# cqf7419/LiDAR-GS

Hardware: AMD Instinct MI355X
Metric: LiDAR range-view frames/sec (fwd+bwd) (higher is better)
Workload: dtype f32

## Files before the change

### lidar-gs_amd/csrc/api.hip

```cpp
#include "lidargs_common.h"
#include "../../include/lidargs_rasterizer.h"

#include <math.h>
#include <stdio.h>
#include <stdlib.h>
#include <string.h>
#include <limits>
#include <algorithm>
#include <mutex>

namespace {
using lg::SegPlan;

thread_local char g_err[512] = "";
thread_local long long g_counters[10] = {0, 0, 0, 0, 0, 0, 0, 0, -1, -1};
thread_local int g_counters_on = 0;
struct CounterPage {
    unsigned long long* dev = nullptr; unsigned long long* host = nullptr; hipEvent_t done = nullptr; int device = -1; bool pending = false;
    bool ready() {
        int d = -1;
        if (hipGetDevice(&d) != hipSuccess) return false;
        if (dev && d == device) return true;
        if (dev) { (void)hipFree(dev); dev = nullptr; }
        if (done) { (void)hipEventDestroy(done); done = nullptr; }
// ... 435 lines not shown
    lg::BinnedFrame bf;
    const int rendered = lg::bin_frame(spec, geom, img.ranges, (size_t)P, width, height, col_lo, col_hi, pp.compact != 0, binning_alloc, binning_user,
                                       debug, stream, &bf);
    if (rendered < 0) return rendered;
    const lg::FrameLayout& L = bf.L;
    const lg::BinView& bin = bf.bin;
    const size_t R = bf.R;

    lg::RenderFwdArgs ra;
    ra.fill.cnt = nullptr;
    ra.grid = L.grid; ra.ranges = img.ranges; ra.point_list = bin.val_a; ra.rec = geom.rec; ra.rowspan = geom.rowspan;
    ra.coltab = img.coltab; ra.rowtab = img.rowtab; ra.bg = background; ra.T_in = T_in;
    ra.final_T = img.final_T; ra.T_pass = T_out;
    ra.out_color = out_color; ra.out_depth = out_depth; ra.out_occ = out_occ;
    ra.seg = bin.seg; ra.S = L.S; ra.seg_len = L.plan.seg_len;
    ra.run_pass1 = (L.S > 1 || transmittance_pass || is_shell) ? 1 : 0;
    ra.flags = ra.run_pass1 ? bin.flags : nullptr; ra.R = L.Rp;
    ra.touched = geom.touched;
    ra.transmittance_only = transmittance_pass;
    ra.seg_lo = 0; ra.seg_hi = L.S; ra.front = 0; ra.alive = nullptr;
    int head = 0;
    if (!L.fused && !ra.run_pass1 && R) lg::launch_touch_all(geom.touched, radii, (size_t)P, stream);
    if (L.fused) {
        ra.flags = bin.flags; ra.alive = bin.alive;
        lg::launch_render_fused(ra, stream);
        LG_STAGE_CHECK("render fused");
        lg::prof_mark("render_fused", stream);
    } else {
    if (ra.run_pass1) {
        run_pass1_rounds(ra, L.plan, bin.alive, stream, transmittance_pass ? nullptr : &head);
        LG_STAGE_CHECK("render pass 1");
        lg::prof_mark("render_pass1", stream);
    }
    ra.seg_lo = head; ra.seg_hi = L.S;
    if (!transmittance_pass) {
        lg::launch_render_pass2(ra, stream);
        LG_STAGE_CHECK("render pass 2");
        lg::prof_mark("render_pass2", stream);
    }
    if (L.work_list) ra.fill = lg::work_list(bin);
    lg::launch_render_combine(ra, stream);
    LG_STAGE_CHECK("render combine");
    lg::prof_mark("render_combine", stream);
    }

    lg::RenderBwdArgs v = lg::RenderBwdArgs();
    v.walk.cnt = nullptr; v.grid = L.grid; v.ranges = img.ranges; v.seg = bin.seg; v.S = L.S; v.seg_len = L.plan.seg_len; v.R = L.Rp;
    v.alive = L.gated ? bin.alive : nullptr;
    v.flags = L.flags ? bin.flags : nullptr;
    lg::note_forward((size_t)P, R, L, geom.totals, ra.flags, geom.touched, (R != 0 && !transmittance_pass) ? &v : nullptr, stream);
    return rendered;
}

struct BackMode {
    bool is_shell = false;
    const float* behind = nullptr;
    const float* T_final_global = nullptr;
    int col_lo = -1, col_hi = -1;
};

int backward_impl(int P, int R, const float* background, int width, int height, const float* means3D,
                  const float* colors_precomp, const float* scales, float scale_modifier, const float* rotations,
                  const float* cov3D_precomp, const float* viewmatrix, const float* beams, const int* radii, char* geom_buffer,
                  char* binning_buffer, char* image_buffer, const BackMode& mode, const float* dL_dpix, const float* dL_dout_depth, const float* dL_dout_occ, float* dL_dmean2D,
                  float* dL_dconic, float* dL_dopacity, float* dL_dcolor, float* dL_ddepths, float* dL_dmean3D,
                  float* dL_dsphere_means3D, float* dL_dbasis_u1, float* dL_dbasis_u2, float* dL_dcov3D, float* dL_dscale,
                  float* dL_drot, int debug, hipStream_t stream) {
    (void)colors_precomp; (void)beams;
    const int col_lo = mode.col_lo, col_hi = mode.col_hi;
    if (P < 0 || R < 0 || width <= 0 || height <= 0) return fail(LIDARGS_ERR_INVALID_ARGUMENT, "backward: bad sizes%s");
    if (P == 0) return 0;
    if (!geom_buffer || !binning_buffer || !image_buffer) return fail(LIDARGS_ERR_STATE, "backward: missing forward buffers%s");
    if (!means3D || !viewmatrix || !radii || !dL_dpix || !dL_dout_depth || !dL_dout_occ || !dL_dmean2D ||
        !dL_dopacity || !dL_dcolor || !dL_dmean3D || !dL_dscale || !dL_drot || (cov3D_precomp && !dL_dcov3D))
        return fail(LIDARGS_ERR_INVALID_ARGUMENT, "backward: NULL required pointer%s");

    lg::GeomView geom; lg::geom_carve(geom_buffer, (size_t)P, lg::GAUSS_BUFFERS, &geom);
    if (col_lo >= 0 && (col_lo % LG_TILE_W || col_hi <= col_lo || col_hi > width)) return fail(LIDARGS_ERR_INVALID_ARGUMENT, "backward: bad column wedge%s");
    const lg::FrameLayout L = lg::frame_layout(R, width, height, col_lo, col_hi, mode.is_shell ? lg::FRAME_SHELL : lg::FRAME_GAUSS);
    lg::BinView bin; L.bin_carve(binning_buffer, &bin);
    lg::ImgView img; lg::img_carve(image_buffer, width, height, lg::make_grid(width, height, 4).num_tiles(), &img);
    lg::prof_begin(stream, 1);

    lg::ZeroRows zr;
    zr.add(dL_dmean2D, 4); zr.add(dL_dconic, 4); zr.add(dL_dopacity, 1); zr.add(dL_dcolor, 2); zr.add(dL_ddepths, 1); zr.add(dL_dmean3D, 3);
    zr.add(dL_dsphere_means3D, 3); zr.add(dL_dbasis_u1, 3); zr.add(dL_dbasis_u2, 3); zr.add(dL_dcov3D, 6); zr.add(dL_dscale, 3); zr.add(dL_drot, 4);
    lg::launch_zero_touched(geom.touched, reinterpret_cast<float4*>(geom.gacc), 4, (size_t)P, geom.tlist, geom.tcount, zr, stream);
    lg::prof_mark("bwd_zero", stream);

    lg::RenderBwdArgs rb;
    rb.walk.cnt = nullptr;
    rb.grid = L.grid; rb.ranges = img.ranges; rb.point_list = bin.val_a; rb.rec = geom.rec; rb.rowspan = geom.rowspan;
    rb.coltab = img.coltab; rb.rowtab = img.rowtab; rb.bg = background; rb.final_T = img.final_T;
    rb.seg = bin.seg; rb.S = L.S; rb.seg_len = L.plan.seg_len;
    rb.alive = L.gated ? bin.alive : nullptr;
    rb.flags = L.flags ? bin.flags : nullptr; rb.R = L.Rp;
    rb.T_final_global = mode.T_final_global; rb.behind = mode.behind;
    rb.dL_dpix = dL_dpix; rb.dL_ddepth = dL_dout_depth; rb.dL_docc = dL_dout_occ; rb.gacc = geom.gacc;
    if (L.work_list) rb.walk = lg::work_list(bin);
    lg::launch_render_backward(rb, stream);
    LG_STAGE_CHECK("render backward");
    lg::prof_mark("render_bwd", stream);

    lg::GaussBwdArgs gb;
    gb.P = P; gb.scale_modifier = scale_modifier;
    gb.view = viewmatrix;
    gb.means3D = means3D; gb.scales = scales; gb.rotations = rotations; gb.cov3D_precomp = cov3D_precomp; gb.radii = radii;
    gb.gacc = geom.gacc; gb.tlist = geom.tlist; gb.tcount = geom.tcount;
    gb.dL_dmean2D = dL_dmean2D; gb.dL_dconic = dL_dconic; gb.dL_dopacity = dL_dopacity; gb.dL_dcolor = dL_dcolor;
    gb.dL_ddepths = dL_ddepths; gb.dL_dbasis_u1 = dL_dbasis_u1; gb.dL_dbasis_u2 = dL_dbasis_u2;
    gb.dL_dsphere = dL_dsphere_means3D; gb.dL_dmean3D = dL_dmean3D; gb.dL_dcov3D = dL_dcov3D; gb.dL_dscale = dL_dscale;
    gb.dL_drot = dL_drot;
    lg::launch_gaussian_backward(gb, stream);
    LG_STAGE_CHECK("gaussian backward");
    lg::prof_mark("gaussian_bwd", stream);
    return 0;
}

}

extern "C" {

int lidargs_abi_version(void) { return LIDARGS_ABI_VERSION; }
const char* lidargs_last_error(void) { return g_err; }

int lidargs_forward(lidargs_alloc_fn geometry_alloc, void* geometry_user, lidargs_alloc_fn binning_alloc, void* binning_user,
                    lidargs_alloc_fn image_alloc, void* image_user, int P, int D, int M, const float* background, int width,
                    int height, const float* means3D, const float* shs, const float* colors_precomp, const float* opacities,
                    const float* scales, float scale_modifier, const float* rotations, const float* cov3D_precomp,
                    const float* viewmatrix, const float* projmatrix, const float* cam_pos, const float* beam_inclinations,
                    int prefiltered, int lidar_far, int lidar_near, float* out_color, float* out_depth, float* out_occ,
                    int* radii, int* radii_xy, int debug, void* stream) {
    (void)D; (void)M; (void)shs; (void)projmatrix; (void)cam_pos; (void)prefiltered;
    const float inf = std::numeric_limits<float>::infinity();
    return forward_impl(geometry_alloc, geometry_user, binning_alloc, binning_user, image_alloc, image_user, P, background, width,
                        height, means3D, colors_precomp, opacities, scales, scale_modifier, rotations, cov3D_precomp, viewmatrix,
                        beam_inclinations, (float)lidar_near, (float)lidar_far, -inf, inf, nullptr, 0, out_color, out_depth,
                        out_occ, nullptr, radii, radii_xy, debug, (hipStream_t)stream, FrameMode());
}

int lidargs_forward_enqueue(lidargs_alloc_fn geometry_alloc, void* geometry_user, lidargs_alloc_fn binning_alloc, void* binning_user,
                            lidargs_alloc_fn image_alloc, void* image_user, int P, int D, int M, const float* background, int width,
                            int height, const float* means3D, const float* shs, const float* colors_precomp, const float* opacities,
                            const float* scales, float scale_modifier, const float* rotations, const float* cov3D_precomp,
                            const float* viewmatrix, const float* projmatrix, const float* cam_pos, const float* beam_inclinations,
                            int prefiltered, int lidar_far, int lidar_near, float* out_color, float* out_depth, float* out_occ,
                            int* radii, int* radii_xy, int debug, int instance_capacity, int tile_rows, unsigned* status_host, void* stream) {
    (void)D; (void)M; (void)shs; (void)projmatrix; (void)cam_pos; (void)prefiltered;
    if (instance_capacity <= 0) return fail(LIDARGS_ERR_INVALID_ARGUMENT, "forward_enqueue: instance_capacity must be positive%s");
    const float inf = std::numeric_limits<float>::infinity();
    FrameMode mode;
    mode.instance_capacity = instance_capacity; mode.fixed_tile_rows = tile_rows; mode.status_host = status_host;
    return forward_impl(geometry_alloc, geometry_user, binning_alloc, binning_user, image_alloc, image_user, P, background, width,
                        height, means3D, colors_precomp, opacities, scales, scale_modifier, rotations, cov3D_precomp, viewmatrix,
                        beam_inclinations, (float)lidar_near, (float)lidar_far, -inf, inf, nullptr, 0, out_color, out_depth,
                        out_occ, nullptr, radii, radii_xy, debug, (hipStream_t)stream, mode);
}

int lidargs_backward(int P, int D, int M, int R, const float* background, int width, int height, const float* means3D,
                     const float* shs, const float* colors_precomp, const float* scales, float scale_modifier,
                     const float* rotations, const float* cov3D_precomp, const float* viewmatrix, const float* projmatrix,
                     const float* campos, const float* beam_inclinations, float tan_fovx, float tan_fovy, const int* radii,
                     char* geom_buffer, char* binning_buffer, char* image_buffer, const float* dL_dpix,
                     const float* dL_dout_depth, const float* dL_dout_occ, float* dL_dmean2D, float* dL_dconic,
                     float* dL_dopacity, float* dL_dcolor, float* dL_ddepths, float* dL_dmean3D, float* dL_dsphere_means3D,
                     float* dL_dbasis_u1, float* dL_dbasis_u2, float* dL_dcov3D, float* dL_dsh, float* dL_dscale, float* dL_drot,
                     int debug, void* stream) {
    (void)D; (void)M; (void)shs; (void)projmatrix; (void)campos; (void)tan_fovx; (void)tan_fovy; (void)dL_dsh;
    return backward_impl(P, R, background, width, height, means3D, colors_precomp, scales, scale_modifier, rotations, cov3D_precomp,
                         viewmatrix, beam_inclinations, radii, geom_buffer, binning_buffer, image_buffer, BackMode(), dL_dpix,
                         dL_dout_depth, dL_dout_occ, dL_dmean2D, dL_dconic, dL_dopacity, dL_dcolor, dL_ddepths, dL_dmean3D,
                         dL_dsphere_means3D, dL_dbasis_u1, dL_dbasis_u2, dL_dcov3D, dL_dscale, dL_drot, debug, (hipStream_t)stream);
}

int lidargs_visible_filter(lidargs_alloc_fn geometry_alloc, void* geometry_user, lidargs_alloc_fn binning_alloc, void* binning_user,
                           lidargs_alloc_fn image_alloc, void* image_user, int P, int M, int width, int height,
                           const float* means3D, const float* scales, float scale_modifier, const float* rotations,
                           const float* cov3D_precomp, const float* viewmatrix, const float* projmatrix, const float* cam_pos,
                           const float* beam_inclinations, float tan_fovx, float tan_fovy, int prefiltered, int lidar_far,
                           int lidar_near, int* radii, int* radii_xy, int debug, void* stream_) {
    (void)geometry_alloc; (void)geometry_user; (void)binning_alloc; (void)binning_user; (void)image_alloc; (void)image_user;
    (void)M; (void)projmatrix; (void)cam_pos; (void)tan_fovx; (void)tan_fovy; (void)prefiltered;
    hipStream_t stream = (hipStream_t)stream_;
    if (P < 0 || width <= 0 || height < 2) return fail(LIDARGS_ERR_INVALID_ARGUMENT, "visible_filter: bad sizes%s");
    if (P == 0) return 0;
    if (!means3D || !viewmatrix || !beam_inclinations || !radii)
        return fail(LIDARGS_ERR_INVALID_ARGUMENT, "visible_filter: NULL required pointer%s");
    if (!cov3D_precomp && (!scales || !rotations)) return fail(LIDARGS_ERR_INVALID_ARGUMENT, "visible_filter: need scales+rotations or cov3D_precomp%s");
    const lg::TileGrid grid = lg::make_grid(width, height, lg::tile_rows());
    lg::PreprocessParams pp;
    pp.P = P; pp.W = width; pp.H = height; pp.TH = grid.TH; pp.tiles_x = grid.tiles_x; pp.tiles_y = grid.tiles_y;
    pp.scale_modifier = scale_modifier;
    pp.near_f = (float)lidar_near; pp.far_f = (float)lidar_far;
    pp.shell_lo = -std::numeric_limits<float>::infinity(); pp.shell_hi = std::numeric_limits<float>::infinity();
    pp.tile_x_lo = 0; pp.tile_x_hi = grid.tiles_x; pp.compact = 0; pp.prune = 1;
// ... 251 lines not shown
```

### lidar-gs_amd/csrc/lidargs_common.h

```cpp
#pragma once
#include <hip/hip_runtime.h>
#include <stdint.h>
#include <stddef.h>

#define LG_TILE_W 16
#define LG_WAVE_ROWS 4
#define LG_CHANNELS 2

#define LG_SEG_TPASS 0
#define LG_SEG_C0 1
#define LG_SEG_C1 2
#define LG_SEG_D 3
#define LG_SEG_TEND 4
#define LG_SEG_TBREAK 5
#define LG_SEG_LAST 6
#define LG_SEG_PLANES 7

#define LG_REGION 256

namespace lg {

struct Carver {
    char* p;
    explicit Carver(char* base) : p(base) {}
// ... 306 lines not shown
    patch = patches - 1 - patch;
    return patch >= 0 && seg < S;
#elif defined(LG_PATCH_ORDER) && LG_PATCH_ORDER == 2
    seg = (int)(b / (unsigned)patches); patch = (int)(b % (unsigned)patches);
    return seg < S;
#endif
    return patch < patches && seg < S;
}
inline unsigned segment_grid(int patches, int S) { return (unsigned)patches * ((unsigned)S | 1u); }
#endif


__device__ __forceinline__ int segment_count(uint2 range, int S, int seg_len) {
    const uint32_t L = range.y - range.x;
    const uint32_t want = (L + (uint32_t)seg_len - 1u) / (uint32_t)seg_len;
    return (int)min((uint32_t)S, max(1u, want));
}
__device__ __forceinline__ uint2 segment_range(uint2 range, int St, int seg) {
    const uint32_t L = range.y - range.x;
    const uint32_t len = (L + (uint32_t)St - 1u) / (uint32_t)St;
    const uint32_t a = min(range.y, range.x + (uint32_t)seg * len);
    const uint32_t b = min(range.y, a + len);
    return make_uint2(a, b);
}

#endif

struct RenderFwdArgs {
    TileGrid grid;
    const uint2* ranges; const uint32_t* point_list; const float4* rec; const uint32_t* rowspan;
    const float2* coltab; const float2* rowtab;
    const float* bg;
    const float* T_in;
    float* final_T; float* T_pass;
    float* out_color; float* out_depth; float* out_occ;
    float* seg; int S;
    int seg_len;
    uint8_t* flags; size_t R;
    uint8_t* touched = nullptr;
    int seg_lo, seg_hi;
    int front;
    uint8_t* alive;
    int run_pass1;
    int transmittance_only;
    WorkList fill;
    int walk2;
    float* T_end_out = nullptr;
};
void launch_render_pass1(const RenderFwdArgs& a, hipStream_t s);
void launch_render_pass2(const RenderFwdArgs& a, hipStream_t s);
void launch_render_head(const RenderFwdArgs& a, int head, hipStream_t s);
void launch_render_alive(const RenderFwdArgs& a, hipStream_t s);
void launch_render_combine(const RenderFwdArgs& a, hipStream_t s);
void launch_render_fused(const RenderFwdArgs& a, hipStream_t s);

struct RenderBwdArgs {
    TileGrid grid;
    const uint2* ranges; const uint32_t* point_list; const float4* rec; const uint32_t* rowspan;
    const float2* coltab; const float2* rowtab;
    const float* bg;
    const float* final_T;
    const float* seg; int S; int seg_len;
    const uint8_t* flags; size_t R;
    const uint8_t* alive;
    const float* T_final_global;
    const float* behind;
    const float* dL_dpix; const float* dL_ddepth; const float* dL_docc;
    float* gacc;
    WorkList walk;
};
void launch_render_backward(const RenderBwdArgs& a, hipStream_t s);
void launch_count_backward_entries(const RenderBwdArgs& a, unsigned long long* out, hipStream_t s);
void note_forward(size_t P, size_t R, const FrameLayout& L, const uint32_t* totals, const uint8_t* flags, const uint8_t* touched,
                  const RenderBwdArgs* view, hipStream_t s);

struct GaussBwdArgs {
    int P; float scale_modifier; const float* view;
    const float* means3D; const float* scales; const float* rotations; const float* cov3D_precomp; const int* radii;
    const float* gacc;
    const uint8_t* tlist; const uint16_t* tcount;
    float* dL_dmean2D; float* dL_dconic; float* dL_dopacity; float* dL_dcolor; float* dL_ddepths;
    float* dL_dbasis_u1; float* dL_dbasis_u2;
    float* dL_dsphere; float* dL_dmean3D; float* dL_dcov3D; float* dL_dscale; float* dL_drot;
};
void launch_gaussian_backward(const GaussBwdArgs& a, hipStream_t s);

#ifdef __HIPCC__
typedef float row4 __attribute__((ext_vector_type(4), aligned(4)));
typedef float row3 __attribute__((ext_vector_type(3), aligned(4)));
typedef float row2 __attribute__((ext_vector_type(2), aligned(4)));
#if defined(LG_GB_VARIANT) && LG_GB_VARIANT == 5
__device__ __forceinline__ void put4(float* p, size_t i, float x, float y, float z, float w) { if (x != x || w * 0.f != 0.f) *reinterpret_cast<row4*>(p + 4 * i) = row4{x, y, z, w}; }
__device__ __forceinline__ void put3(float* p, size_t i, float x, float y, float z) { if (x != x || z * 0.f != 0.f) *reinterpret_cast<row3*>(p + 3 * i) = row3{x, y, z}; }
__device__ __forceinline__ void put2(float* p, size_t i, float x, float y) { if (x != x || y * 0.f != 0.f) *reinterpret_cast<row2*>(p + 2 * i) = row2{x, y}; }
#else
__device__ __forceinline__ void put4(float* p, size_t i, float x, float y, float z, float w) { *reinterpret_cast<row4*>(p + 4 * i) = row4{x, y, z, w}; }
__device__ __forceinline__ void put3(float* p, size_t i, float x, float y, float z) { *reinterpret_cast<row3*>(p + 3 * i) = row3{x, y, z}; }
__device__ __forceinline__ void put2(float* p, size_t i, float x, float y) { *reinterpret_cast<row2*>(p + 2 * i) = row2{x, y}; }
#endif
#if defined(LG_GB_VARIANT) && LG_GB_VARIANT == 6
__device__ __forceinline__ float3 get3(const float* p, size_t i) { const float f = 1.f + (float)(i & 1023) * 1e-3f; return make_float3(f, 0.5f * f, 0.25f + f); }
__device__ __forceinline__ float4 get4(const float* p, size_t i) { const float f = 1.f + (float)(i & 1023) * 1e-3f; return make_float4(0.5f, 0.5f * f, 0.5f, 0.5f / f); }
#else
__device__ __forceinline__ float3 get3(const float* p, size_t i) { const row3 v = *reinterpret_cast<const row3*>(p + 3 * i); return make_float3(v.x, v.y, v.z); }
__device__ __forceinline__ float4 get4(const float* p, size_t i) { const row4 v = *reinterpret_cast<const row4*>(p + 4 * i); return make_float4(v.x, v.y, v.z, v.w); }
#endif

typedef float v4f __attribute__((ext_vector_type(4)));
typedef float v3f __attribute__((ext_vector_type(3)));
#define LG_LDS_VOLATILE(T) const volatile __attribute__((address_space(3))) T*
__device__ __forceinline__ float4 lds_ahead(const float4* p) {
    const v4f v = *(LG_LDS_VOLATILE(v4f))p;
    return make_float4(v.x, v.y, v.z, v.w);
}
__device__ __forceinline__ float lds_ahead(const float* p) { return *(LG_LDS_VOLATILE(float))p; }
__device__ __forceinline__ uint32_t lds_ahead(const uint32_t* p) { return *(LG_LDS_VOLATILE(uint32_t))p; }

__device__ __forceinline__ float fold_halves32(float a, float b) {
    const auto r = __builtin_amdgcn_permlane32_swap(__float_as_uint(a), __float_as_uint(b), false, false);
    return __uint_as_float(r[0]) + __uint_as_float(r[1]);
}
__device__ __forceinline__ float fold_halves16(float a, float b) {
    const auto r = __builtin_amdgcn_permlane16_swap(__float_as_uint(a), __float_as_uint(b), false, false);
    return __uint_as_float(r[0]) + __uint_as_float(r[1]);
}

__device__ __forceinline__ float plane_product(float T, const float* first, size_t stride, int n) {
    int k = 0;
    for (; k + 8 <= n; k += 8) {
        float x[8];
#pragma unroll
        for (int i = 0; i < 8; i++) x[i] = first[(size_t)(k + i) * stride];
#pragma unroll
        for (int i = 0; i < 8; i++) T *= x[i];
    }
    float x[8];
#pragma unroll
    for (int i = 0; i < 8; i++) x[i] = (k + i < n) ? first[(size_t)(k + i) * stride] : 1.f;
#pragma unroll
    for (int i = 0; i < 8; i++) if (k + i < n) T *= x[i];
    return T;
}
template <int NP>
__device__ __forceinline__ void plane_sums(float (&acc)[NP], const float* first, size_t stride, const int (&plane)[NP], int n) {
    int k = 0;
    for (; k + 4 <= n; k += 4) {
        float x[4][NP];
#pragma unroll
        for (int i = 0; i < 4; i++)
#pragma unroll
            for (int p = 0; p < NP; p++) x[i][p] = first[(size_t)(k + i) * stride + (size_t)plane[p] * 64];
#pragma unroll
        for (int i = 0; i < 4; i++)
#pragma unroll
            for (int p = 0; p < NP; p++) acc[p] += x[i][p];
    }
    for (; k < n; k++)
#pragma unroll
        for (int p = 0; p < NP; p++) acc[p] += first[(size_t)k * stride + (size_t)plane[p] * 64];
}

__device__ __forceinline__ float4 rows_opacity(uint32_t span, float opacity, int y0) {
    const int lo = (int)(span & 0xFFFFu), hi = (int)(span >> 16);
    float4 o;
    o.x = (y0 >= lo && y0 < hi) ? opacity : 0.f;
    o.y = (y0 + 1 >= lo && y0 + 1 < hi) ? opacity : 0.f;
// ... 8 lines not shown
```

### lidar-gs_amd/csrc/preprocess.hip

```cpp
#include "lidargs_common.h"
#include "selection.h"
#include <algorithm>

namespace lg {

__device__ __forceinline__ float3 f3(float x, float y, float z) { return make_float3(x, y, z); }
__device__ __forceinline__ float dot3(float3 a, float3 b) { return a.x * b.x + a.y * b.y + a.z * b.z; }
__device__ __forceinline__ float3 scale3(float3 a, float s) { return f3(a.x * s, a.y * s, a.z * s); }
__device__ __forceinline__ float3 add3(float3 a, float3 b) { return f3(a.x + b.x, a.y + b.y, a.z + b.z); }

__device__ __forceinline__ float3 view_to_world(const float* vm, float3 v) {
    return f3(vm[0] * v.x + vm[1] * v.y + vm[2] * v.z,
              vm[4] * v.x + vm[5] * v.y + vm[6] * v.z,
              vm[8] * v.x + vm[9] * v.y + vm[10] * v.z);
}
__device__ __forceinline__ float3 world_to_view_dir(const float* vm, float3 v) {
    return f3(vm[0] * v.x + vm[4] * v.y + vm[8] * v.z,
              vm[1] * v.x + vm[5] * v.y + vm[9] * v.z,
              vm[2] * v.x + vm[6] * v.y + vm[10] * v.z);
}

struct Sym3 { float xx, xy, xz, yy, yz, zz; };
__device__ __forceinline__ float3 symmul(const Sym3& S, float3 v) {
    return f3(S.xx * v.x + S.xy * v.y + S.xz * v.z,
// ... 243 lines not shown
    {
        __shared__ uint32_t s_part[4][8];
        uint32_t s4 = t4, s8 = t8, s16 = t16, s32 = t32, sv = reftiles ? 1u : 0u, sr = reftiles;
        uint32_t kinv = ~key, kmx = (key == 0xFFFFFFFFu) ? 0u : key;
#pragma unroll
        for (int o = 32; o > 0; o >>= 1) {
            s4 += __shfl_xor(s4, o); s8 += __shfl_xor(s8, o); s16 += __shfl_xor(s16, o); s32 += __shfl_xor(s32, o);
            sv += __shfl_xor(sv, o); sr += __shfl_xor(sr, o);
            kinv = max(kinv, (uint32_t)__shfl_xor((int)kinv, o)); kmx = max(kmx, (uint32_t)__shfl_xor((int)kmx, o));
        }
        if ((threadIdx.x & 63) == 0) {
            uint32_t* q = s_part[threadIdx.x >> 6];
            q[0] = s4; q[1] = s8; q[2] = s16; q[3] = s32; q[4] = sv; q[5] = sr; q[6] = kinv; q[7] = kmx;
        }
        __syncthreads();
        if (threadIdx.x == 6 || threadIdx.x == 7) {
            const int c = threadIdx.x;
            const uint32_t m = max(max(s_part[0][c], s_part[1][c]), max(s_part[2][c], s_part[3][c]));
            if (m) atomicMax(a.key_span + 2 * (size_t)(blockIdx.x % LG_INST_SLOTS) + (c - 6), m);
        }
        if (threadIdx.x < 6) {
            const uint32_t sum = s_part[0][threadIdx.x] + s_part[1][threadIdx.x] + s_part[2][threadIdx.x] + s_part[3][threadIdx.x];
            const size_t slot = (size_t)(blockIdx.x % LG_INST_SLOTS);
            if (sum) {
                if (threadIdx.x < 4) atomicAdd(a.inst_slots + slot * 4 + threadIdx.x, (unsigned long long)sum);
                else atomicAdd(a.diag_slots + slot * 2 + (threadIdx.x - 4), (unsigned long long)sum);
            }
        }
    }
    if (!in_range) return;
    a.touched[idx] = 0;
    a.dkey[idx] = key;
    if (pp.compact) reinterpret_cast<uint32_t*>(a.spans)[idx] = span_pack(rspan, tiles ? xsp : 0u);
    else a.spans[idx] = make_uint4(rspan, tiles ? xsp : 0u, 0u, 0u);
    if (live && tiles) {
        a.rowspan[idx] = rspan;
        float4* r = a.rec + 4 * (size_t)idx;
        r[0] = r0; r[1] = r1; r[2] = r2; r[3] = r3;
    }
}

void launch_preprocess(const PreprocessParams& pp, const float* means3D, const float* scales, const float* rotations,
                       const float* opacities, const float* colors, const float* cov3D_precomp, const float* beams,
                       int* radii, int* radii_xy, GeomView g, const ImgView* tables, bool filter_only, hipStream_t s) {
    PreKernelArgs a;
    a.pp = pp;
    a.means3D = means3D; a.scales = scales; a.rotations = rotations; a.opacities = opacities; a.colors = colors;
    a.cov3D_precomp = cov3D_precomp; a.beams = beams; a.radii = radii; a.radii_xy = radii_xy;
    a.coltab = tables ? tables->coltab : nullptr; a.rowtab = tables ? tables->rowtab : nullptr;
    a.rec = g.rec; a.rowspan = g.rowspan; a.spans = g.spans; a.dkey = g.key_a; a.ids = g.id_a;
    a.touched = g.touched;
    a.inst_slots = reinterpret_cast<unsigned long long*>(g.totals + LG_TOTALS_SLOT_WORD);
    a.diag_slots = reinterpret_cast<unsigned long long*>(g.totals + LG_TOTALS_DIAG_WORD);
    a.key_span = g.totals + LG_TOTALS_KEYSPAN_WORD;
    const dim3 grid((pp.P + 255) / 256), block(256);
    if (filter_only) hipLaunchKernelGGL(k_preprocess<true>, grid, block, 0, s, a);
    else hipLaunchKernelGGL(k_preprocess<false>, grid, block, 0, s, a);
}

__global__ void k_mark_visible(int P, const float* __restrict__ means3D, const float* __restrict__ vm, unsigned char* __restrict__ present) {
    const int i = blockIdx.x * blockDim.x + threadIdx.x;
    if (i >= P) return;
    const float x = means3D[3 * i], y = means3D[3 * i + 1], z = means3D[3 * i + 2];
    const float vz = vm[2] * x + vm[6] * y + vm[10] * z + vm[14];
    present[i] = (vz <= 0.2f) ? 0 : 1;
}

void launch_mark_visible(int P, const float* means3D, const float* view, unsigned char* present, hipStream_t s) {
    hipLaunchKernelGGL(k_mark_visible, dim3((P + 255) / 256), dim3(256), 0, s, P, means3D, view, present);
}

__global__ void k_debug_rects(int n, int surfel, const float2* __restrict__ p, const int2* __restrict__ r, int gx, int gy, int4* __restrict__ out) {
    const int i = blockIdx.x * blockDim.x + threadIdx.x;
    if (i >= n) return;
    int xmin, ymin, xmax, ymax;
    if (surfel) rect_surfel(p[i].x, p[i].y, r[i].x, r[i].y, gx, gy, xmin, ymin, xmax, ymax);
    else rect_lidar(p[i].x, p[i].y, r[i].x, r[i].y, gx, gy, xmin, ymin, xmax, ymax);
    out[i] = make_int4(xmin, ymin, xmax, ymax);
}
void launch_debug_rects(int n, int surfel, const float* p_cr, const int* r_xy, int gx, int gy, int* rects, hipStream_t s) {
    k_debug_rects<<<(n + 255) / 256, 256, 0, s>>>(n, surfel, (const float2*)p_cr, (const int2*)r_xy, gx, gy, (int4*)rects);
}

__device__ __forceinline__ void gb_row(const GaussBwdArgs& a, const int idx) {
#pragma clang fp contract(fast)
    const float* vm = a.view;

    const float3 pw = get3(a.means3D, idx);
    const float4* acc = reinterpret_cast<const float4*>(a.gacc) + 4 * (size_t)idx;
#if defined(LG_GB_VARIANT) && LG_GB_VARIANT == 7
    const float ff = (float)(idx & 255);
    const float4 q0 = make_float4(ff, 1.f, 2.f, ff), q1 = q0, q2 = q0, q3 = q0;
#else
    const float4 q0 = acc[0], q1 = acc[1], q2 = acc[2], q3 = acc[3];
#endif
    const bool have_sr = (a.cov3D_precomp == nullptr);
    float3 s_in = f3(0, 0, 0); float4 q = make_float4(1, 0, 0, 0);
    float3 cv0 = f3(0, 0, 0), cv1 = f3(0, 0, 0);
    if (have_sr || a.scales) { s_in = get3(a.scales, idx); q = get4(a.rotations, idx); }
    if (!have_sr) { cv0 = get3(a.cov3D_precomp, 2 * (size_t)idx); cv1 = get3(a.cov3D_precomp, 2 * (size_t)idx + 1); }
    const float3 d = f3(vm[0] * pw.x + vm[4] * pw.y + vm[8] * pw.z + vm[12],
                        vm[1] * pw.x + vm[5] * pw.y + vm[9] * pw.z + vm[13],
                        vm[2] * pw.x + vm[6] * pw.y + vm[10] * pw.z + vm[14]);
    const float n2 = d.x * d.x + d.y * d.y + d.z * d.z;
    const float dist = __builtin_amdgcn_sqrtf(n2);
    if (dist <= 0.f) return;
    auto frcp = [](float b) { const float r = __builtin_amdgcn_rcpf(b); return __builtin_fmaf(__builtin_fmaf(-b, r, 1.f), r, r); };
    const float inv_dist = frcp(dist);
    const float3 dir = f3(d.x * inv_dist, d.y * inv_dist, d.z * inv_dist);
    float3 u1, u2;
    tangent_basis(dir, u1, u2);

    Sym3 S;
    const float3 sc = f3(a.scale_modifier * s_in.x, a.scale_modifier * s_in.y, a.scale_modifier * s_in.z);
    if (!have_sr) { S.xx = cv0.x; S.xy = cv0.y; S.xz = cv0.z; S.yy = cv1.x; S.yz = cv1.y; S.zz = cv1.z; }
    else S = covariance_world(sc, q);
    const float3 t1 = view_to_world(vm, u1), t2 = view_to_world(vm, u2);
    const float3 St1 = symmul(S, t1), St2 = symmul(S, t2);
    const float _a = dot3(t1, St1) + 0.01f, _b = dot3(t1, St2), _c = dot3(t2, St2) + 0.01f;
    const float inv_d2 = frcp(dist * dist);
    const float ca = inv_d2 * _a, cb = inv_d2 * _b, cc = inv_d2 * _c;

    const float gx = q0.x, gy = q0.y;
    const float gA = q0.w, gB = q1.x, gC = q1.y;
    const float gdep = q2.y;
    float3 du1, du2;
    {
        const float w1 = dot3(u1, u1), w2 = dot3(u2, u2);
        const float j1 = w1 > 0.f ? frcp(w1) : 0.f, j2 = w2 > 0.f ? frcp(w2) : 0.f;
        const float3 G1 = f3(q2.z, q2.w, q3.x), G2 = f3(q3.y, q3.z, q3.w);
        const float3 p1 = scale3(u1, j1), p2 = scale3(u2, j2);
        const float c1 = 2.f * dot3(p1, G1), c2 = 2.f * dot3(p2, G2);
        du1 = f3(j1 * G1.x - c1 * p1.x, j1 * G1.y - c1 * p1.y, j1 * G1.z - c1 * p1.z);
        du2 = f3(j2 * G2.x - c2 * p2.x, j2 * G2.y - c2 * p2.y, j2 * G2.z - c2 * p2.z);
    }
    put4(a.dL_dmean2D, idx, gx, gy, q0.z, 0.f);
    if (a.dL_dconic) put4(a.dL_dconic, idx, gA, gB, 0.f, gC);
    a.dL_dopacity[idx] = q1.z;
    put2(a.dL_dcolor, idx, q1.w, q2.x);
    if (a.dL_ddepths) a.dL_ddepths[idx] = gdep;
    if (a.dL_dbasis_u1) put3(a.dL_dbasis_u1, idx, du1.x, du1.y, du1.z);
    if (a.dL_dbasis_u2) put3(a.dL_dbasis_u2, idx, du2.x, du2.y, du2.z);

    const float denom = __fsub_rn(__fmul_rn(ca, cc), __fmul_rn(cb, cb));
    const float k = frcp((denom * denom) + 0.0000001f);
    float da = k * (-cc * cc * gA + 2.f * cb * cc * gB + (denom - ca * cc) * gC);
    float dc = k * (-ca * ca * gC + 2.f * ca * cb * gB + (denom - ca * cc) * gA);
    float db = k * 2.f * (cb * cc * gA - (denom + 2.f * cb * cb) * gB + ca * cb * gC);
    const float dist4 = n2 * n2;
    const float wsum = -2.f * (da * _a + db * _b + dc * _c) * frcp(dist4);
    float3 g_mean = f3(wsum * d.x, wsum * d.y, wsum * d.z);
    da *= inv_d2; dc *= inv_d2; db *= inv_d2;

    const float S00 = t1.x * t1.x * da + t1.x * t2.x * db + t2.x * t2.x * dc;
    const float S11 = t1.y * t1.y * da + t1.y * t2.y * db + t2.y * t2.y * dc;
    const float S22 = t1.z * t1.z * da + t1.z * t2.z * db + t2.z * t2.z * dc;
    const float S01 = 2.f * t1.x * t1.y * da + (t1.x * t2.y + t1.y * t2.x) * db + 2.f * t2.x * t2.y * dc;
    const float S02 = 2.f * t1.x * t1.z * da + (t1.x * t2.z + t1.z * t2.x) * db + 2.f * t2.x * t2.z * dc;
    const float S12 = 2.f * t1.z * t1.y * da + (t1.y * t2.z + t1.z * t2.y) * db + 2.f * t2.y * t2.z * dc;
    if (a.dL_dcov3D) { put3(a.dL_dcov3D, 2 * (size_t)idx, S00, S01, S02); put3(a.dL_dcov3D, 2 * (size_t)idx + 1, S11, S12, S22); }

    const float3 gt1 = add3(scale3(St1, 2.f * da), scale3(St2, db));
    const float3 gt2 = add3(scale3(St2, 2.f * dc), scale3(St1, db));
    float3 gu1 = world_to_view_dir(vm, gt1), gu2 = world_to_view_dir(vm, gt2);
    gu1.x += du1.x; gu1.y += du1.y;
    gu2.x += du2.x; gu2.y += du2.y; gu2.z += du2.z;

    const float rho2 = dir.x * dir.x + dir.y * dir.y;
    const float srho = __builtin_amdgcn_sqrtf(rho2);
    const float i32 = frcp((float)((double)(srho * srho * srho) + 1e-9));
    const float irho = frcp((float)((double)srho + 1e-9));
    float3 gdir;
    gdir.x = i32 * (-dir.y * dir.x * gu1.x - dir.y * dir.y * gu1.y + dir.z * dir.y * dir.y * gu2.x - dir.x * dir.y * dir.z * gu2.y) - dir.x * irho * gu2.z;
    gdir.y = i32 * (dir.x * dir.x * gu1.x + dir.x * dir.y * gu1.y - dir.x * dir.y * dir.z * gu2.x + dir.z * dir.x * dir.x * gu2.y) - dir.y * irho * gu2.z;
    gdir.z = irho * (dir.x * gu2.x + dir.y * gu2.y);
    const float d3 = dist * dist * dist;
    const float id3e = frcp((float)((double)d3 + 1e-9));
    const float dg = dot3(d, gdir);
    g_mean = add3(g_mean, scale3(f3(n2 * gdir.x - d.x * dg, n2 * gdir.y - d.y * dg, n2 * gdir.z - d.z * dg), id3e));

    const float uu1 = dot3(u1, u1), uu2 = dot3(u2, u2);
    const float i1 = uu1 > 0.f ? frcp(uu1) : 0.f, i2 = uu2 > 0.f ? frcp(uu2) : 0.f;
    const float3 gs = add3(scale3(u1, gx * i1), scale3(u2, gy * i2));
    if (a.dL_dsphere) put3(a.dL_dsphere, idx, gs.x, gs.y, gs.z);
    const float id3 = frcp(d3);
    const float dgs = dot3(d, gs);
    float3 v;
    v.x = g_mean.x + (n2 * gs.x - d.x * dgs) * id3 + gdep * dir.x;
    v.y = g_mean.y + (n2 * gs.y - d.y * dgs) * id3 + gdep * dir.y;
    v.z = g_mean.z + (n2 * gs.z - d.z * dgs) * id3 + gdep * dir.z;
    const float3 gw = view_to_world(vm, v);
    put3(a.dL_dmean3D, idx, gw.x, gw.y, gw.z);

    if (!a.scales) {
        put3(a.dL_dscale, idx, 0.f, 0.f, 0.f);
        put4(a.dL_drot, idx, 0.f, 0.f, 0.f, 0.f);
    } else {
        Sym3 G; G.xx = S00; G.xy = 0.5f * S01; G.xz = 0.5f * S02; G.yy = S11; G.yz = 0.5f * S12; G.zz = S22;
        float3 c0, c1, c2;
        quat_columns(q, c0, c1, c2);
        const float3 h0 = symmul(G, c0), h1 = symmul(G, c1), h2 = symmul(G, c2);
        put3(a.dL_dscale, idx, 2.f * sc.x * dot3(c0, h0), 2.f * sc.y * dot3(c1, h1), 2.f * sc.z * dot3(c2, h2));
        const float3 F0 = scale3(h0, 2.f * sc.x * sc.x), F1 = scale3(h1, 2.f * sc.y * sc.y), F2 = scale3(h2, 2.f * sc.z * sc.z);
        const float F00 = F0.x, F01 = F0.y, F02 = F0.z, F10 = F1.x, F11 = F1.y, F12 = F1.z, F20 = F2.x, F21 = F2.y, F22 = F2.z;
        const float r = q.x, x = q.y, y = q.z, z = q.w;
        put4(a.dL_drot, idx, 2.f * z * (F01 - F10) + 2.f * y * (F20 - F02) + 2.f * x * (F12 - F21),
             2.f * y * (F10 + F01) + 2.f * z * (F20 + F02) + 2.f * r * (F12 - F21) - 4.f * x * (F22 + F11),
             2.f * x * (F10 + F01) + 2.f * r * (F20 - F02) + 2.f * z * (F12 + F21) - 4.f * y * (F22 + F00),
             2.f * r * (F01 - F10) + 2.f * x * (F20 + F02) + 2.f * y * (F12 + F21) - 4.f * z * (F11 + F00));
    }
}

__global__ void __launch_bounds__(256) k_gaussian_backward(const GaussBwdArgs a) {
    const int lane = threadIdx.x & 63;
    const int region = blockIdx.x * 4 + (threadIdx.x >> 6);
    const int base = region * LG_REGION;
    if (base >= a.P) return;
    int off = (int)a.tlist[base + lane];
    int cnt = (int)a.tcount[region];
    asm volatile("" : "+v"(off), "+v"(cnt));
    for (int j = lane; j < cnt; j += 64) {
        gb_row(a, base + off);
        if (j + 64 < cnt) off = (int)a.tlist[base + j + 64];
    }
}

template <int LINE>
__global__ void __launch_bounds__(LG_REGION) k_zero_touched(const uint8_t* __restrict__ touched, float4* __restrict__ acc, size_t P,
                                                           uint8_t* __restrict__ tlist, uint16_t* __restrict__ tcount, const ZeroRows zr) {
    __shared__ uint32_t s_wcnt[LG_REGION / 64];
    const int tid = threadIdx.x, lane = tid & 63, wv = tid >> 6;
    const size_t base = (size_t)blockIdx.x * LG_REGION;
    const size_t i = base + tid;
    const bool mark = i < P && touched[i] != 0;
    const unsigned long long m0 = __ballot(mark);
    if (lane == 0) s_wcnt[wv] = (uint32_t)__popcll(m0);
    {
        unsigned long long m = m0;
        const size_t wbase = i - (size_t)lane;
        constexpr int PER = 64 / LINE;
        const int sub = lane / LINE, part = lane % LINE;
        const float4 z = make_float4(0.f, 0.f, 0.f, 0.f);
        while (m) {
            unsigned long long mm = m;
            int mine = -1;
#pragma unroll
            for (int k = 0; k < PER; k++) {
                const int j = mm ? __builtin_ctzll(mm) : -1;
                if (k == sub) mine = j;
                mm &= mm - 1ull;
            }
            m = mm;
            if (mine >= 0) acc[(wbase + (size_t)mine) * LINE + part] = z;
        }
    }
    if (i < P) {
        for (int k = 0; k < zr.n; k++) {
            float* q = zr.p[k];
            switch (zr.w[k]) {
                case 1: q[i] = 0.f; break;
                case 2: put2(q, i, 0.f, 0.f); break;
                case 3: put3(q, i, 0.f, 0.f, 0.f); break;
                case 4: put4(q, i, 0.f, 0.f, 0.f, 0.f); break;
                case 6: put3(q, 2 * i, 0.f, 0.f, 0.f); put3(q, 2 * i + 1, 0.f, 0.f, 0.f); break;
                default: for (int c = 0; c < zr.w[k]; c += 3) put3(q, (size_t)(zr.w[k] / 3) * i + c / 3, 0.f, 0.f, 0.f); break;
            }
        }
    }
    __syncthreads();
    uint32_t off = 0, total = 0;
#pragma unroll
    for (int v = 0; v < LG_REGION / 64; v++) { off += v < wv ? s_wcnt[v] : 0u; total += s_wcnt[v]; }
    if (mark) tlist[base + off + (uint32_t)__popcll(m0 & ((1ull << lane) - 1ull))] = (uint8_t)tid;
    if (tid == 0) tcount[blockIdx.x] = (uint16_t)total;
}
void launch_zero_touched(const uint8_t* touched, float4* acc, int line_f4, size_t P, uint8_t* tlist, uint16_t* tcount, const ZeroRows& zr, hipStream_t s) {
    const unsigned blocks = (unsigned)((P + LG_REGION - 1) / LG_REGION);
    if (!blocks) return;
    if (line_f4 == 8) hipLaunchKernelGGL(k_zero_touched<8>, dim3(blocks), dim3(LG_REGION), 0, s, touched, acc, P, tlist, tcount, zr);
    else hipLaunchKernelGGL(k_zero_touched<4>, dim3(blocks), dim3(LG_REGION), 0, s, touched, acc, P, tlist, tcount, zr);
}
__global__ void __launch_bounds__(256) k_touch_visible(uint8_t* __restrict__ touched, const int* __restrict__ radii, size_t P) {
    const size_t i = (size_t)blockIdx.x * 256 + threadIdx.x;
    if (i < P) touched[i] = radii[i] > 0 ? 1 : 0;
}
void launch_touch_all(uint8_t* touched, const int* radii, size_t P, hipStream_t s) {
    hipLaunchKernelGGL(k_touch_visible, dim3((unsigned)((P + 255) / 256)), dim3(256), 0, s, touched, radii, P);
}

void launch_gaussian_backward(const GaussBwdArgs& a, hipStream_t s) {
    const unsigned regions = (unsigned)((a.P + LG_REGION - 1) / LG_REGION);
    hipLaunchKernelGGL(k_gaussian_backward, dim3((regions + 3) / 4), dim3(256), 0, s, a);
}

}
```

Baseline: 1531.

## Defer zeroing of gradient output rows into the gaussian backward kernel

Zeroing of the per-Gaussian gradient output arrays moves out of the zero_touched kernel and into the gaussian backward kernel. Each wave zeroes its whole region span with vectorized float4 stores, then computes and writes the touched rows, using a wavefront release fence to order those writes after the zeros. The first row's inputs are loaded before the zeroing so that load latency overlaps the stores. This keeps the zero stores off the critical path before render backward, but it relies on intra-wave ordering of overlapping stores. An env var can turn the old behaviour back on.

Result: faster. 1556, median of 6 (+1.6%).

```diff
diff --git a/lidar-gs_amd/csrc/api.hip b/lidar-gs_amd/csrc/api.hip
--- a/lidar-gs_amd/csrc/api.hip
+++ b/lidar-gs_amd/csrc/api.hip
@@ -541,10 +541,11 @@
     lg::ImgView img; lg::img_carve(image_buffer, width, height, lg::make_grid(width, height, 4).num_tiles(), &img);
     lg::prof_begin(stream, 1);
 
+    static const bool rows_late = [] { const char* e = getenv("LIDARGS_BWD_ROWS"); return !e || atoi(e) != 0; }();
     lg::ZeroRows zr;
     zr.add(dL_dmean2D, 4); zr.add(dL_dconic, 4); zr.add(dL_dopacity, 1); zr.add(dL_dcolor, 2); zr.add(dL_ddepths, 1); zr.add(dL_dmean3D, 3);
     zr.add(dL_dsphere_means3D, 3); zr.add(dL_dbasis_u1, 3); zr.add(dL_dbasis_u2, 3); zr.add(dL_dcov3D, 6); zr.add(dL_dscale, 3); zr.add(dL_drot, 4);
-    lg::launch_zero_touched(geom.touched, reinterpret_cast<float4*>(geom.gacc), 4, (size_t)P, geom.tlist, geom.tcount, zr, stream);
+    lg::launch_zero_touched(geom.touched, reinterpret_cast<float4*>(geom.gacc), 4, (size_t)P, geom.tlist, geom.tcount, rows_late ? lg::ZeroRows() : zr, stream);
     lg::prof_mark("bwd_zero", stream);
 
     lg::RenderBwdArgs rb;
@@ -570,6 +571,7 @@
     gb.dL_ddepths = dL_ddepths; gb.dL_dbasis_u1 = dL_dbasis_u1; gb.dL_dbasis_u2 = dL_dbasis_u2;
     gb.dL_dsphere = dL_dsphere_means3D; gb.dL_dmean3D = dL_dmean3D; gb.dL_dcov3D = dL_dcov3D; gb.dL_dscale = dL_dscale;
     gb.dL_drot = dL_drot;
+    if (rows_late) gb.rows = zr;
     lg::launch_gaussian_backward(gb, stream);
     LG_STAGE_CHECK("gaussian backward");
     lg::prof_mark("gaussian_bwd", stream);
diff --git a/lidar-gs_amd/csrc/lidargs_common.h b/lidar-gs_amd/csrc/lidargs_common.h
--- a/lidar-gs_amd/csrc/lidargs_common.h
+++ b/lidar-gs_amd/csrc/lidargs_common.h
@@ -412,6 +412,7 @@
     float* dL_dmean2D; float* dL_dconic; float* dL_dopacity; float* dL_dcolor; float* dL_ddepths;
     float* dL_dbasis_u1; float* dL_dbasis_u2;
     float* dL_dsphere; float* dL_dmean3D; float* dL_dcov3D; float* dL_dscale; float* dL_drot;
+    ZeroRows rows;
 };
 void launch_gaussian_backward(const GaussBwdArgs& a, hipStream_t s);
 
diff --git a/lidar-gs_amd/csrc/preprocess.hip b/lidar-gs_amd/csrc/preprocess.hip
--- a/lidar-gs_amd/csrc/preprocess.hip
+++ b/lidar-gs_amd/csrc/preprocess.hip
@@ -349,29 +349,40 @@
     k_debug_rects<<<(n + 255) / 256, 256, 0, s>>>(n, surfel, (const float2*)p_cr, (const int2*)r_xy, gx, gy, (int4*)rects);
 }
 
-__device__ __forceinline__ void gb_row(const GaussBwdArgs& a, const int idx) {
-#pragma clang fp contract(fast)
-    const float* vm = a.view;
-
-    const float3 pw = get3(a.means3D, idx);
+struct GbIn { float3 pw; float4 q0, q1, q2, q3; float3 s_in; float4 q; float3 cv0, cv1; };
+__device__ __forceinline__ GbIn gb_load(const GaussBwdArgs& a, const int idx) {
+    GbIn in;
+    in.pw = get3(a.means3D, idx);
     const float4* acc = reinterpret_cast<const float4*>(a.gacc) + 4 * (size_t)idx;
 #if defined(LG_GB_VARIANT) && LG_GB_VARIANT == 7
     const float ff = (float)(idx & 255);
-    const float4 q0 = make_float4(ff, 1.f, 2.f, ff), q1 = q0, q2 = q0, q3 = q0;
+    in.q0 = make_float4(ff, 1.f, 2.f, ff); in.q1 = in.q0; in.q2 = in.q0; in.q3 = in.q0;
 #else
-    const float4 q0 = acc[0], q1 = acc[1], q2 = acc[2], q3 = acc[3];
+    in.q0 = acc[0]; in.q1 = acc[1]; in.q2 = acc[2]; in.q3 = acc[3];
 #endif
     const bool have_sr = (a.cov3D_precomp == nullptr);
-    float3 s_in = f3(0, 0, 0); float4 q = make_float4(1, 0, 0, 0);
-    float3 cv0 = f3(0, 0, 0), cv1 = f3(0, 0, 0);
-    if (have_sr || a.scales) { s_in = get3(a.scales, idx); q = get4(a.rotations, idx); }
-    if (!have_sr) { cv0 = get3(a.cov3D_precomp, 2 * (size_t)idx); cv1 = get3(a.cov3D_precomp, 2 * (size_t)idx + 1); }
+    in.s_in = f3(0, 0, 0); in.q = make_float4(1, 0, 0, 0);
+    in.cv0 = f3(0, 0, 0); in.cv1 = f3(0, 0, 0);
+    if (have_sr || a.scales) { in.s_in = get3(a.scales, idx); in.q = get4(a.rotations, idx); }
+    if (!have_sr) { in.cv0 = get3(a.cov3D_precomp, 2 * (size_t)idx); in.cv1 = get3(a.cov3D_precomp, 2 * (size_t)idx + 1); }
+    return in;
+}
+template <bool AFTER_ZEROS>
+__device__ __forceinline__ void gb_row(const GaussBwdArgs& a, const int idx, const GbIn& in) {
+#pragma clang fp contract(fast)
+    const float* vm = a.view;
+    const float3 pw = in.pw;
+    const float4 q0 = in.q0, q1 = in.q1, q2 = in.q2, q3 = in.q3;
+    const bool have_sr = (a.cov3D_precomp == nullptr);
+    const float3 s_in = in.s_in; const float4 q = in.q;
+    const float3 cv0 = in.cv0, cv1 = in.cv1;
     const float3 d = f3(vm[0] * pw.x + vm[4] * pw.y + vm[8] * pw.z + vm[12],
                         vm[1] * pw.x + vm[5] * pw.y + vm[9] * pw.z + vm[13],
                         vm[2] * pw.x + vm[6] * pw.y + vm[10] * pw.z + vm[14]);
     const float n2 = d.x * d.x + d.y * d.y + d.z * d.z;
     const float dist = __builtin_amdgcn_sqrtf(n2);
     if (dist <= 0.f) return;
+    if (AFTER_ZEROS) __builtin_amdgcn_fence(__ATOMIC_RELEASE, "wavefront");
     auto frcp = [](float b) { const float r = __builtin_amdgcn_rcpf(b); return __builtin_fmaf(__builtin_fmaf(-b, r, 1.f), r, r); };
     const float inv_dist = frcp(dist);
     const float3 dir = f3(d.x * inv_dist, d.y * inv_dist, d.z * inv_dist);
@@ -478,6 +489,16 @@
     }
 }
 
+__device__ __forceinline__ void zero_span(float* q, const int n, const int lane) {
+    const int head = min(n, (int)((0u - (uint32_t)(reinterpret_cast<uintptr_t>(q) >> 2)) & 3u));
+    if (lane < head) q[lane] = 0.f;
+    float4* v = reinterpret_cast<float4*>(q + head);
+    const int nv = (n - head) >> 2, tail = (n - head) & 3;
+    const float4 z = make_float4(0.f, 0.f, 0.f, 0.f);
+    for (int i = lane; i < nv; i += 64) v[i] = z;
+    if (lane < tail) q[head + 4 * nv + lane] = 0.f;
+}
+template <bool ROWS_HERE>
 __global__ void __launch_bounds__(256) k_gaussian_backward(const GaussBwdArgs a) {
     const int lane = threadIdx.x & 63;
     const int region = blockIdx.x * 4 + (threadIdx.x >> 6);
@@ -486,9 +507,21 @@
     int off = (int)a.tlist[base + lane];
     int cnt = (int)a.tcount[region];
     asm volatile("" : "+v"(off), "+v"(cnt));
-    for (int j = lane; j < cnt; j += 64) {
-        gb_row(a, base + off);
+    const bool first = lane < cnt;
+    GbIn in;
+    if (first) in = gb_load(a, base + off);
+    const int idx0 = base + off;
+    if (lane + 64 < cnt) off = (int)a.tlist[base + lane + 64];
+    if (ROWS_HERE) {
+        asm volatile("" ::: "memory");
+        const int rows = min(LG_REGION, a.P - base);
+        for (int k = 0; k < a.rows.n; k++) zero_span(a.rows.p[k] + (size_t)base * a.rows.w[k], rows * a.rows.w[k], lane);
+    }
+    if (first) gb_row<ROWS_HERE>(a, idx0, in);
+    for (int j = lane + 64; j < cnt; j += 64) {
+        const int idx = base + off;
         if (j + 64 < cnt) off = (int)a.tlist[base + j + 64];
+        gb_row<ROWS_HERE>(a, idx, gb_load(a, idx));
     }
 }
 
@@ -557,7 +590,8 @@
 
 void launch_gaussian_backward(const GaussBwdArgs& a, hipStream_t s) {
     const unsigned regions = (unsigned)((a.P + LG_REGION - 1) / LG_REGION);
-    hipLaunchKernelGGL(k_gaussian_backward, dim3((regions + 3) / 4), dim3(256), 0, s, a);
-}
-
-}
+    if (a.rows.n) hipLaunchKernelGGL(k_gaussian_backward<true>, dim3((regions + 3) / 4), dim3(256), 0, s, a);
+    else hipLaunchKernelGGL(k_gaussian_backward<false>, dim3((regions + 3) / 4), dim3(256), 0, s, a);
+}
+
+}
```
